# HuiGuanLab/Lite-MKD

Measured on AMD Instinct MI355X. Metric: episodes/sec (5-way 5-shot, 8x224^2 frames), higher is better.
Workload: dtype f32

## Files before the change

### include/lmkd.h

```cpp
#ifndef LMKD_H
#define LMKD_H
#ifdef __cplusplus
extern "C" {
#endif

int lmkd_abi_version(void);
const char* lmkd_last_error(void);
int lmkd_device_check(int device);
int lmkd_set_activation_dtype(int mode);
int lmkd_get_activation_dtype(void);

int lmkd_gemm_f32(char layA, char layB, int M, int N, int K, float alpha, const float* A, long lda, long sA,
                  const float* B, long ldb, long sB, float beta, float* C, long ldc, long sC, const float* bias,
                  int relu, int batch, void* stream);
int lmkd_gemm_set_mode(int mode);
int lmkd_gemm_set_tile(int t);
long lmkd_gemm_ticket_words(void);
int lmkd_gemm_f32_splitk(char layA, char layB, int M, int N, int K, float alpha, const float* A, long lda, long sA,
                         const float* B, long ldb, long sB, float beta, float* C, long ldc, long sC, const float* bias,
                         int relu, int batch, void* workspace, long ws_bytes, unsigned* tickets, void* stream);

long lmkd_conv2d_packed_weight_elems(int Cout, int Cin, int Cs, int KH, int KW, int mode);
int lmkd_conv2d_pack_weights(const float* w_oihw, float* wp, int Cout, int Cin, int Cs, int KH, int KW, int mode ,
                             void* stream);
int lmkd_conv2d_fwd_row_tiles(int N, int H, int W, int Cout, int KH, int KW, int stride, int pad);
int lmkd_conv2d_fwd_row_tiles_cs(int N, int H, int W, int Cs, int Cout, int KH, int KW, int stride, int pad);
int lmkd_set_elementwise_wg_per_cu(int n);
int lmkd_conv_set_compute_dtype(int mode);
typedef struct lmkd_amax_desc {
  const void* x_words;
  const void* dy_words;
  void* out_words;
  const void* ref_words;
  int flags;
} lmkd_amax_desc;
#define LMKD_AMAX_FENCED 1
int lmkd_h2_fence_eval(const void* const* words, void* const* refs, int n, int* flags, void* stream);
long lmkd_conv_h2_fallbacks(void);
int lmkd_amax(const float* x, long n, void* word, void* stream);
long lmkd_amax_words(void);
long lmkd_conv2d_plane_elems(int ncols, int Kp);
long lmkd_conv_h2_launches(void);
int lmkd_conv2d_repack_multi(const float* const* ws, void* const* wfs, const int* dims, int n, void* stream);
int lmkd_conv2d_split_weights(const float* wp, void* wf, int ncols, int Kp, void* stream);
int lmkd_conv_get_compute_dtype(void);
int lmkd_conv_set_wgrad_planes(int on);
int lmkd_conv_set_patch(int on);
int lmkd_conv_set_stem_patch(int on);
int lmkd_conv_set_s2_patch(int on);
int lmkd_conv_set_wgrad_win16(int on);
int lmkd_conv_set_wgrad_stem(int on);
int lmkd_conv_set_wgrad_window(int on);
int lmkd_conv_set_patch16(int on);
int lmkd_conv_set_persistent(int on);
int lmkd_conv_set_xcd_mode(int mode);
int lmkd_conv_set_tile(int id);
int lmkd_conv2d_fwd(const float* x, const float* wp_fwd, float* y, float* stat_partial, int N, int H, int W, int Cs, int Cout,
                    int KH, int KW, int stride, int pad, void* stream);
int lmkd_conv2d_fwd_pre(const float* x_raw, const float* pre_stats, const float* wp_fwd, float* y, float* stat_partial, int N, int H,
                        int W, int Cs, int Cout, int KH, int KW, int stride, int pad, void* stream);
int lmkd_conv2d_fwd_bn(const float* x, const float* wp_fwd, float* y, const float* bn_stats, const float* res , int relu,
                       int N, int H, int W, int Cs, int Cout, int KH, int KW, int stride, int pad, void* stream,
                       const lmkd_amax_desc* amax );
int lmkd_conv2d_bwd_data(const float* dy, const float* wp_dgrad, float* dx, int N, int H, int W, int Cin, int Cout, int KH, int KW,
                         int stride, int pad, int accumulate, void* stream);
int lmkd_conv2d_bwd_data_bn_tiles(int N, int H, int W, int Cin, int Cout, int KH, int KW, int stride, int pad);
int lmkd_conv2d_bwd_data_bn(const float* dy, const float* wp_dgrad, float* dx, const float* bn_x, const float* bn_stats, float* part,
                            int N, int H, int W, int Cin, int Cout, int KH, int KW, int stride, int pad, void* stream);
long lmkd_conv2d_bwd_weight_workspace(int N, int H, int W, int Cs, int Cout, int KH, int KW, int stride, int pad);
int lmkd_conv2d_bwd_weight(const float* x, const float* dy, float* dw_oihw, float* workspace, long ws_bytes, int N, int H, int W,
                           int Cs, int Cin, int Cout, int KH, int KW, int stride, int pad, void* stream);
int lmkd_conv2d_bwd_weight_pre(const float* x_raw, const float* pre_stats, const float* dy, float* dw_oihw, float* workspace,
                               long ws_bytes, int N, int H, int W, int Cs, int Cin, int Cout, int KH, int KW, int stride, int pad,
                               void* stream);

int lmkd_conv2d_plan(int kind, int N, int H, int W, int Cs, int Cin, int Cout, int KH, int KW, int stride, int pad, int* info_host);

int lmkd_conv2d_bwd_weight_acc(const float* x, const float* pre_stats, const float* dy, float* dw_oihw, float* workspace, long ws_bytes,
                               int N, int H, int W, int Cs, int Cin, int Cout, int KH, int KW, int stride, int pad, void* stream);

int lmkd_frames_u8_to_nhwc4(const unsigned char* src, float* dst, const int* crop_y, const int* crop_x, const int* flip, int F, int Hs,
                            int Ws, int H, int W, int frames_per_video, void* stream);
int lmkd_resize_plan(int in_size, int out_size, int* bounds_host, int* coeffs_host);
int lmkd_resize_pass_u8(const unsigned char* src, unsigned char* dst, const int* bounds_dev, const int* coeffs_dev, int ksize, long outer,
                        int n_in, int n_out, long inner, void* stream);
int lmkd_frames_resize_crop_nhwc4(const unsigned char* src, float* dst, const int* bounds_h, const int* coeffs_h, int ksize_h,
                                  const int* bounds_v, const int* coeffs_v, int ksize_v, const int* crop_y, const int* crop_x,
                                  const int* flip, int F, int Hs, int Ws, int Hr, int Wr, int H, int W, int frames_per_video, void* stream);
long lmkd_jpeg_desc_bytes(void);
long lmkd_jpeg_pool_bytes(int n);
const char* lmkd_jpeg_reason(int reason);
int lmkd_jpeg_plan(const unsigned char* data, const long long* offsets, int n, void* descs, void* pool, long pool_cap, long long* info,
                   long long* totals);
int lmkd_jpeg_decode(const unsigned char* data, const void* descs, const void* pool, int n, short* coef, unsigned char* planes,
                     unsigned char* out, int* status, long long max_blocks, long long max_pixels, void* stream);
int lmkd_jpeg_decode_host(const unsigned char* data, const void* descs, const void* pool, int n, short* coef, unsigned char* planes,
                          unsigned char* out, int* status);
int lmkd_nchw3_to_nhwc4(const float* x_nchw, float* y_nhwc4, int N, int H, int W, void* stream, void* amax_words);
long lmkd_ticket_words(void);
// ... 190 lines not shown
```

### lite-mkd_amd/csrc/gemm.hip

```cpp
#include "gemm_core.h"

struct GemmArgs {
  const float* A;
  const float* B;
  float* C;
  const float* bias;
  long lda, ldb, ldc;
  long sA, sB, sC;
  int M, N, K;
  float alpha, beta;
  int relu;
  int splits, k_per;
  float* ws;
  unsigned* tickets;
};

template <class Cfg, bool A_KMAJOR, bool B_KMAJOR>
__global__ __launch_bounds__(LMKD_THREADS) void gemm_kernel(GemmArgs g) {
  using LA = typename std::conditional<A_KMAJOR, LoaderKMajorDense<Cfg::BM>, LoaderMMajorDense<Cfg::BM>>::type;
  using LB = typename std::conditional<B_KMAJOR, LoaderKMajorDense<Cfg::BN>, LoaderMMajorDense<Cfg::BN>>::type;
  __shared__ __attribute__((aligned(16))) float smem[2 * (LA::LDS_FLOATS + LB::LDS_FLOATS)];
  __shared__ int s_last;
  const int m0 = blockIdx.x * Cfg::BM, n0 = blockIdx.y * Cfg::BN;
  const int S = g.splits;
  const long bz = S > 1 ? blockIdx.z / S : blockIdx.z;
  const int ks = S > 1 ? (int)(blockIdx.z - bz * S) : 0;
  const int k0 = ks * g.k_per;
  const int k1 = S > 1 ? (k0 + g.k_per < g.K ? k0 + g.k_per : g.K) : g.K;
  LA la;
  LB lb;
  la.init(g.A + bz * g.sA, g.lda, m0, g.M, k1);
  lb.init(g.B + bz * g.sB, g.ldb, n0, g.N, k1);
  f32x16 acc[Cfg::TM][Cfg::TN];
  const int nk = (k1 - k0 + LMKD_BK - 1) / LMKD_BK;
  auto koff = [k0](int t) { return k0 + t * LMKD_BK; };
  gemm_mainloop<Cfg>(la, lb, nk, koff, koff, smem, acc);

  const int lane = threadIdx.x & 63, wave = threadIdx.x >> 6;
  const int wm = wave / Cfg::WN, wn = wave % Cfg::WN;
  if (S > 1) {
    float* wp = g.ws + (bz * S + ks) * (long)g.M * g.N;
#pragma unroll
    for (int j = 0; j < Cfg::TN; ++j) {
      const int col = n0 + wn * (Cfg::TN * 32) + j * 32 + (lane & 31);
      if (col >= g.N) continue;
#pragma unroll
      for (int i = 0; i < Cfg::TM; ++i)
#pragma unroll
        for (int e = 0; e < 16; ++e) {
          const int row = m0 + wm * (Cfg::TM * 32) + i * 32 + acc_row(e, lane);
          if (row < g.M) __hip_atomic_store(wp + (long)row * g.N + col, acc[i][j][e], __ATOMIC_RELAXED, __HIP_MEMORY_SCOPE_AGENT);
        }
    }
    asm volatile("s_waitcnt vmcnt(0)" ::: "memory");
    __syncthreads();
    unsigned* tk = g.tickets + (bz * gridDim.y + blockIdx.y) * gridDim.x + blockIdx.x;
    if (threadIdx.x == 0) s_last = atomicAdd(tk, 1u) == (unsigned)(S - 1);
    __syncthreads();
    if (!s_last) return;
    asm volatile("" ::: "memory");
    const float* w0 = g.ws + bz * S * (long)g.M * g.N;
#pragma unroll
    for (int j = 0; j < Cfg::TN; ++j) {
      const int col = n0 + wn * (Cfg::TN * 32) + j * 32 + (lane & 31);
#pragma unroll
      for (int i = 0; i < Cfg::TM; ++i)
#pragma unroll
        for (int e = 0; e < 16; ++e) acc[i][j][e] = 0.f;
      if (col >= g.N) continue;
      for (int q = 0; q < S; ++q) {
        const float* wq = w0 + (long)q * g.M * g.N;
#pragma unroll
        for (int i = 0; i < Cfg::TM; ++i)
#pragma unroll
          for (int e = 0; e < 16; ++e) {
            const int row = m0 + wm * (Cfg::TM * 32) + i * 32 + acc_row(e, lane);
            if (row < g.M) acc[i][j][e] += __hip_atomic_load(wq + (long)row * g.N + col, __ATOMIC_RELAXED, __HIP_MEMORY_SCOPE_AGENT);
          }
      }
    }
    if (threadIdx.x == 0) *tk = 0u;
  }
  float* C = g.C + bz * g.sC;
#pragma unroll
  for (int j = 0; j < Cfg::TN; ++j) {
    const int col = n0 + wn * (Cfg::TN * 32) + j * 32 + (lane & 31);
    if (col >= g.N) continue;
    const float bv = g.bias ? g.bias[col] : 0.f;
#pragma unroll
    for (int i = 0; i < Cfg::TM; ++i) {
#pragma unroll
      for (int e = 0; e < 16; ++e) {
        const int row = m0 + wm * (Cfg::TM * 32) + i * 32 + acc_row(e, lane);
        if (row < g.M) {
          float* c = C + (long)row * g.ldc + col;
          float v = g.alpha * acc[i][j][e] + bv;
          if (g.beta != 0.f) v += g.beta * *c;
          if (g.relu) v = fmaxf(v, 0.f);
          *c = v;
        }
      }
    }
  }
}

#include "gemm_x3.h"

static int g_gemm_mode = -1;
static int g_gemm_tile = 0;
extern "C" int lmkd_gemm_set_tile(int t) { g_gemm_tile = t; return LMKD_OK; }
extern "C" int lmkd_gemm_set_mode(int mode) {
  LMKD_REQUIRE(mode >= -1 && mode <= 2, "lmkd_gemm_set_mode: -1 follow the convolutions, 0 fp32 MFMA, 1 fp32 as 3 x bf16, 2 bf16");
  g_gemm_mode = mode;
  return LMKD_OK;
}
extern "C" int lmkd_conv_get_compute_dtype(void);
static inline int gemm_planes(int M, int N, int K) {
  int m = g_gemm_mode;
  if (m < 0) m = lmkd_conv_get_compute_dtype() == 0 ? 0 : 1;
  if (m == 0 || (long)M * N * K < (1L << 18)) return 0;
  return m == 2 ? 1 : 3;
}

template <class Cfg>
static int launch_gemm(const GemmArgs& g, int batch, int ak, int bk, hipStream_t s) {
  dim3 grid(cdiv(g.M, Cfg::BM), cdiv(g.N, Cfg::BN), batch * (g.splits > 1 ? g.splits : 1));
  if (ak && bk) hipLaunchKernelGGL((gemm_kernel<Cfg, true, true>), grid, dim3(LMKD_THREADS), 0, s, g);
  else if (ak && !bk) hipLaunchKernelGGL((gemm_kernel<Cfg, true, false>), grid, dim3(LMKD_THREADS), 0, s, g);
  else if (!ak && bk) hipLaunchKernelGGL((gemm_kernel<Cfg, false, true>), grid, dim3(LMKD_THREADS), 0, s, g);
  else hipLaunchKernelGGL((gemm_kernel<Cfg, false, false>), grid, dim3(LMKD_THREADS), 0, s, g);
  LMKD_CHECK_LAUNCH("lmkd_gemm_f32");
  return LMKD_OK;
}

#define LMKD_GEMM_TICKET_WORDS 4096
extern "C" long lmkd_gemm_ticket_words(void) { return LMKD_GEMM_TICKET_WORDS; }

static void gemm_split_plan(int M, int N, int K, int batch, long ws_bytes, int* splits, int* k_per) {
  *splits = 1;
  *k_per = K;
  const long tiles = (long)cdiv(M, 64) * cdiv(N, 64) * batch;
  if (tiles > 64 || K < 256) return;
  int S = (int)cdiv(768, tiles);
  if (S > 16) S = 16;
  if (S > K / 128) S = K / 128;
  const long per = (long)M * N * batch * sizeof(float);
  if ((long)S * per > ws_bytes) S = (int)(ws_bytes / per);
  if (S < 2) return;
  int kp = cdiv(cdiv(K, S), LMKD_BK) * LMKD_BK;
  *k_per = kp;
  *splits = cdiv(K, kp);
  if (*splits < 2) { *splits = 1; *k_per = K; }
}

static int gemm_impl(char layA, char layB, int M, int N, int K, float alpha, const float* A, long lda, long sA, const float* B, long ldb,
                     long sB, float beta, float* C, long ldc, long sC, const float* bias, int relu, int batch, void* workspace,
                     long ws_bytes, unsigned* tickets, void* stream) {
  LMKD_REQUIRE(layA == 'K' || layA == 'M', "lmkd_gemm_f32: layA must be 'K' or 'M'");
  LMKD_REQUIRE(layB == 'K' || layB == 'N', "lmkd_gemm_f32: layB must be 'K' or 'N'");
  LMKD_REQUIRE(M > 0 && N > 0 && K > 0 && batch > 0, "lmkd_gemm_f32: empty problem M=%d N=%d K=%d batch=%d", M, N, K, batch);
  LMKD_REQUIRE(A && B && C, "lmkd_gemm_f32: null operand");
  LMKD_REQUIRE(aligned16(A) && aligned16(B), "lmkd_gemm_f32: operands must be 16-byte aligned");
  LMKD_REQUIRE(lda % 4 == 0 && ldb % 4 == 0 && sA % 4 == 0 && sB % 4 == 0, "lmkd_gemm_f32: lda/ldb/strides must be multiples of 4");
  if (layA == 'K') LMKD_REQUIRE(K % 4 == 0, "lmkd_gemm_f32: K %% 4 != 0 with K-major A");
  else LMKD_REQUIRE(M % 4 == 0, "lmkd_gemm_f32: M %% 4 != 0 with K-outer A");
  if (layB == 'K') LMKD_REQUIRE(K % 4 == 0, "lmkd_gemm_f32: K %% 4 != 0 with K-major B");
  else LMKD_REQUIRE(N % 4 == 0, "lmkd_gemm_f32: N %% 4 != 0 with K-outer B");
  GemmArgs g;
  g.A = A; g.B = B; g.C = C; g.bias = bias;
  g.lda = lda; g.ldb = ldb; g.ldc = ldc; g.sA = sA; g.sB = sB; g.sC = sC;
  g.M = M; g.N = N; g.K = K; g.alpha = alpha; g.beta = beta; g.relu = relu;
  g.splits = 1; g.k_per = K; g.ws = (float*)workspace; g.tickets = tickets;
  if (workspace && tickets) gemm_split_plan(M, N, K, batch, ws_bytes, &g.splits, &g.k_per);
  hipStream_t s = (hipStream_t)stream;
  const int ak = layA == 'K', bk = layB == 'K';
  const long t128 = (long)cdiv(M, 128) * cdiv(N, 128) * batch;
  if (g.splits == 1) {
    if (const int npl = gemm_planes(M, N, K)) {
      if (g_gemm_tile == 1) return npl == 3 ? launch_gemm_x3<G3Cfg<128, 128, 2, 2>, 3>(g, batch, ak, bk, s) : launch_gemm_x3<G3Cfg<128, 128, 2, 2>, 1>(g, batch, ak, bk, s);
      if (g_gemm_tile == 2) return npl == 3 ? launch_gemm_x3<G3Cfg<64, 128, 1, 4>, 3>(g, batch, ak, bk, s) : launch_gemm_x3<G3Cfg<64, 128, 1, 4>, 1>(g, batch, ak, bk, s);
      return npl == 3 ? launch_gemm_x3<G3Cfg<64, 64, 2, 2>, 3>(g, batch, ak, bk, s) : launch_gemm_x3<G3Cfg<64, 64, 2, 2>, 1>(g, batch, ak, bk, s);
    }
  }
  if (t128 >= 384) return launch_gemm<TileCfg<128, 128, 2, 2>>(g, batch, ak, bk, s);
  return launch_gemm<TileCfg<64, 64, 2, 2>>(g, batch, ak, bk, s);
}

extern "C" int lmkd_gemm_f32(char layA, char layB, int M, int N, int K, float alpha, const float* A, long lda,
                             long sA, const float* B, long ldb, long sB, float beta, float* C, long ldc, long sC,
                             const float* bias, int relu, int batch, void* stream) {
  return gemm_impl(layA, layB, M, N, K, alpha, A, lda, sA, B, ldb, sB, beta, C, ldc, sC, bias, relu, batch, nullptr, 0, nullptr, stream);
}

extern "C" int lmkd_gemm_f32_splitk(char layA, char layB, int M, int N, int K, float alpha, const float* A, long lda, long sA,
                                    const float* B, long ldb, long sB, float beta, float* C, long ldc, long sC, const float* bias,
                                    int relu, int batch, void* workspace, long ws_bytes, unsigned* tickets, void* stream) {
  LMKD_REQUIRE(workspace && tickets && ws_bytes > 0, "lmkd_gemm_f32_splitk: workspace / tickets missing");
  LMKD_REQUIRE(aligned16(workspace), "lmkd_gemm_f32_splitk: workspace must be 16-byte aligned");
  return gemm_impl(layA, layB, M, N, K, alpha, A, lda, sA, B, ldb, sB, beta, C, ldc, sC, bias, relu, batch, workspace, ws_bytes, tickets, stream);
}
```

### lite-mkd_amd/csrc/gemm_core.h

```cpp
#pragma once
#include "common.h"
#include <type_traits>

#define LMKD_BK 32
#define LMKD_THREADS 256

struct Tap {
  int dh, dw, kofs;
};
#define LMKD_MAX_TAPS 9
#define LMKD_MAX_CLASSES 4

template <int BM_, int BN_, int WM_, int WN_>
struct TileCfg {
  static constexpr int BM = BM_, BN = BN_, WM = WM_, WN = WN_;
  static constexpr int TM = BM / WM / 32, TN = BN / WN / 32;
  static constexpr int THREADS = 64 * WM * WN;
  static_assert(WM * WN == 4 || WM * WN == 8, "4 or 8 waves");
  static_assert(TM >= 1 && TN >= 1, "wave tile");
};

#define LMKD_LDK 36

template <int ROWS, int THREADS = LMKD_THREADS>
// ... 114 lines not shown

typedef __bf16 bf16x8 __attribute__((ext_vector_type(8)));

template <bool ROWK, int LD, int N>
__device__ __forceinline__ void read_frags_bf16(const float* __restrict__ S, int row, int h, int m, bf16x8 (&f)[N]) {
#pragma unroll
  for (int i = 0; i < N; ++i) {
    float v[8];
    if (ROWK) {
      const float4 q0 = *reinterpret_cast<const float4*>(S + (row + 32 * i) * LD + 16 * m + 8 * h);
      const float4 q1 = *reinterpret_cast<const float4*>(S + (row + 32 * i) * LD + 16 * m + 8 * h + 4);
      v[0] = q0.x; v[1] = q0.y; v[2] = q0.z; v[3] = q0.w; v[4] = q1.x; v[5] = q1.y; v[6] = q1.z; v[7] = q1.w;
    } else {
#pragma unroll
      for (int j = 0; j < 8; ++j) v[j] = S[(16 * m + 8 * h + j) * LD + row + 32 * i];
    }
#pragma unroll
    for (int j = 0; j < 8; ++j) f[i][j] = (__bf16)v[j];
  }
}

template <class Cfg, class LA, class LB>
__device__ __forceinline__ void mfma_kstep_bf16(const float* __restrict__ As, const float* __restrict__ Bs, int a_row, int b_row,
                                                int h, f32x16 (&acc)[Cfg::TM][Cfg::TN]) {
  constexpr int NM = LMKD_BK / 16;
  bf16x8 a[2][Cfg::TM], b[2][Cfg::TN];
  read_frags_bf16<LA::ROWK, LA::LD, Cfg::TM>(As, a_row, h, 0, a[0]);
  read_frags_bf16<LB::ROWK, LB::LD, Cfg::TN>(Bs, b_row, h, 0, b[0]);
#pragma unroll
  for (int m = 0; m < NM; ++m) {
    const int cur = m & 1, nxt = cur ^ 1;
    if (m + 1 < NM) {
      read_frags_bf16<LA::ROWK, LA::LD, Cfg::TM>(As, a_row, h, m + 1, a[nxt]);
      read_frags_bf16<LB::ROWK, LB::LD, Cfg::TN>(Bs, b_row, h, m + 1, b[nxt]);
    }
#pragma unroll
    for (int i = 0; i < Cfg::TM; ++i)
#pragma unroll
      for (int jj = 0; jj < Cfg::TN; ++jj)
        acc[i][jj] = __builtin_amdgcn_mfma_f32_32x32x16_bf16(a[cur][i], b[cur][jj], acc[i][jj], 0, 0, 0);
  }
}

template <class Cfg, class LA, class LB, class FA, class FB, bool BF16 = false, bool FENCE_STORE = false>
__device__ __forceinline__ void gemm_mainloop(LA& la, LB& lb, int nk, FA koffA, FB koffB, float* smem,
                                              f32x16 (&acc)[Cfg::TM][Cfg::TN]) {
  constexpr int SA = LA::LDS_FLOATS, SB = LB::LDS_FLOATS;
  float* As0 = smem;
  float* Bs0 = smem + 2 * SA;
  const int lane = threadIdx.x & 63, wave = threadIdx.x >> 6;
  const int wm = wave / Cfg::WN, wn = wave % Cfg::WN;
  const int h = lane >> 5;
  const int a_row = wm * (Cfg::TM * 32) + (lane & 31);
  const int b_row = wn * (Cfg::TN * 32) + (lane & 31);
#pragma unroll
  for (int i = 0; i < Cfg::TM; ++i)
#pragma unroll
    for (int j = 0; j < Cfg::TN; ++j)
#pragma unroll
      for (int e = 0; e < 16; ++e) acc[i][j][e] = 0.f;
  if (nk <= 0) return;
  la.load(koffA(0));
  lb.load(koffB(0));
  la.store(As0);
  lb.store(Bs0);
  __syncthreads();
  for (int t = 0; t + 1 < nk; ++t) {
    const int cur = t & 1;
    la.load(koffA(t + 1));
    lb.load(koffB(t + 1));
    if (BF16) mfma_kstep_bf16<Cfg, LA, LB>(As0 + cur * SA, Bs0 + cur * SB, a_row, b_row, h, acc);
    else mfma_kstep<Cfg, LA, LB>(As0 + cur * SA, Bs0 + cur * SB, a_row, b_row, h, acc);
    __builtin_amdgcn_sched_barrier(0);
    (void)FENCE_STORE;
    la.store(As0 + (cur ^ 1) * SA);
    lb.store(Bs0 + (cur ^ 1) * SB);
    __syncthreads();
  }
  const int last = (nk - 1) & 1;
  if (BF16) mfma_kstep_bf16<Cfg, LA, LB>(As0 + last * SA, Bs0 + last * SB, a_row, b_row, h, acc);
  else mfma_kstep<Cfg, LA, LB>(As0 + last * SA, Bs0 + last * SB, a_row, b_row, h, acc);
}

__device__ __forceinline__ int acc_row(int e, int lane) { return (e & 3) + 8 * (e >> 2) + 4 * (lane >> 5); }
```

### lite-mkd_amd/csrc/gemm_x3.h

```cpp
#pragma once

typedef short g3_s16x4 __attribute__((ext_vector_type(4)));
#define G3_LD 40

__device__ __forceinline__ unsigned g3_hi2(unsigned x1, unsigned x0) { return __builtin_amdgcn_perm(x1, x0, 0x07060302u); }

template <int NPL>
__device__ __forceinline__ void g3_split_store(unsigned char* d, int plane_bytes, const float4& v) {
  if (NPL == 1) {
    union { __bf16 h[4]; uint2 u; } c;
    c.h[0] = (__bf16)v.x; c.h[1] = (__bf16)v.y; c.h[2] = (__bf16)v.z; c.h[3] = (__bf16)v.w;
    *reinterpret_cast<uint2*>(d) = c.u;
    return;
  }
  const float x[4] = {v.x, v.y, v.z, v.w};
  unsigned b0[4], b1[4], b2[4];
#pragma unroll
  for (int j = 0; j < 4; ++j) {
    b0[j] = __float_as_uint(x[j]);
    const float r1 = x[j] - __uint_as_float(b0[j] & 0xffff0000u);
    b1[j] = __float_as_uint(r1);
    const float r2 = r1 - __uint_as_float(b1[j] & 0xffff0000u);
    b2[j] = __float_as_uint(r2);
  }
  *reinterpret_cast<uint2*>(d) = make_uint2(g3_hi2(b0[1], b0[0]), g3_hi2(b0[3], b0[2]));
  *reinterpret_cast<uint2*>(d + plane_bytes) = make_uint2(g3_hi2(b1[1], b1[0]), g3_hi2(b1[3], b1[2]));
  *reinterpret_cast<uint2*>(d + 2 * plane_bytes) = make_uint2(g3_hi2(b2[1], b2[0]), g3_hi2(b2[3], b2[2]));
}

template <int ROWS, bool KMAJOR, int NPL>
struct G3Img {
  static constexpr int LDB = KMAJOR ? G3_LD * 2 : ROWS * 2 + 64;
  static constexpr int PLANE = KMAJOR ? ROWS * LDB : LMKD_BK * LDB;
  static constexpr int BYTES = NPL * PLANE;
  static_assert(KMAJOR || (LDB / 64) % 2 == 1, "K-outer row stride must be an odd multiple of 64 bytes");
  template <class L>
  static __device__ __forceinline__ void store(unsigned char* img, const L& l) {
    const int tid = threadIdx.x;
#pragma unroll
    for (int i = 0; i < L::NI; ++i) {
      if constexpr (KMAJOR) g3_split_store<NPL>(img + (((tid >> 3) + L::RPP * i) * G3_LD + l.kc4) * 2, PLANE, l.reg[i]);
      else g3_split_store<NPL>(img + (tid / L::CPR + L::KPP * i) * LDB + l.r4 * 2, PLANE, l.reg[i]);
    }
  }
  static __device__ __forceinline__ int lane_off(int row0, int lane) {
    if (KMAJOR) return ((row0 + (lane & 31)) * G3_LD + 8 * (lane >> 5)) * 2;
    const int idx = lane & 15;
    return (8 * (lane >> 5) + (idx >> 2)) * LDB + (row0 + 16 * ((lane >> 4) & 1) + 4 * (idx & 3)) * 2;
  }
  static __device__ __forceinline__ bf16x8 frag(const unsigned char* img, int off, int i, int g, int p) {
    if (KMAJOR) return *reinterpret_cast<const bf16x8*>(img + off + p * PLANE + i * (32 * LDB) + g * 32);
    const unsigned char* a = img + off + p * PLANE + g * 16 * LDB + i * 64;
    const g3_s16x4 lo = __builtin_amdgcn_ds_read_tr16_b64_v4i16((g3_s16x4 __attribute__((address_space(3)))*)a);
    const g3_s16x4 hi = __builtin_amdgcn_ds_read_tr16_b64_v4i16((g3_s16x4 __attribute__((address_space(3)))*)(a + 4 * LDB));
    union { g3_s16x4 s[2]; bf16x8 b; } u;
    u.s[0] = lo; u.s[1] = hi;
    return u.b;
  }
};

template <int BM_, int BN_, int WM_, int WN_>
struct G3Cfg {
  static constexpr int BM = BM_, BN = BN_, WM = WM_, WN = WN_;
  static constexpr int TM = BM / WM / 32, TN = BN / WN / 32;
  static_assert(WM * WN == 4 && TM >= 1 && TN >= 1, "4 waves");
};

template <class Cfg, bool A_KMAJOR, bool B_KMAJOR, int NPL>
__global__ __launch_bounds__(LMKD_THREADS) void gemm_x3_kernel(GemmArgs g) {
  using LA = typename std::conditional<A_KMAJOR, LoaderKMajorDense<Cfg::BM>, LoaderMMajorDense<Cfg::BM>>::type;
  using LB = typename std::conditional<B_KMAJOR, LoaderKMajorDense<Cfg::BN>, LoaderMMajorDense<Cfg::BN>>::type;
  using IA = G3Img<Cfg::BM, A_KMAJOR, NPL>;
  using IB = G3Img<Cfg::BN, B_KMAJOR, NPL>;
  __shared__ __attribute__((aligned(16))) unsigned char smem[IA::BYTES + IB::BYTES];
  unsigned char* sa = smem;
  unsigned char* sb = smem + IA::BYTES;
  const int m0 = blockIdx.x * Cfg::BM, n0 = blockIdx.y * Cfg::BN;
  const long bz = blockIdx.z;
  LA la;
  LB lb;
  la.init(g.A + bz * g.sA, g.lda, m0, g.M, g.K);
  lb.init(g.B + bz * g.sB, g.ldb, n0, g.N, g.K);
  const int lane = threadIdx.x & 63, wave = threadIdx.x >> 6;
  const int wm = wave / Cfg::WN, wn = wave % Cfg::WN;
  const int offA = IA::lane_off(wm * (Cfg::TM * 32), lane), offB = IB::lane_off(wn * (Cfg::TN * 32), lane);
  f32x16 acc[Cfg::TM][Cfg::TN];
#pragma unroll
  for (int i = 0; i < Cfg::TM; ++i)
#pragma unroll
    for (int j = 0; j < Cfg::TN; ++j)
#pragma unroll
      for (int e = 0; e < 16; ++e) acc[i][j][e] = 0.f;
  unsigned sgn[Cfg::TM];
#pragma unroll
  for (int i = 0; i < Cfg::TM; ++i)
    sgn[i] = (NPL == 3 && (((m0 >> 5) + wm * Cfg::TM + i + (n0 >> 5) + wn * Cfg::TN) & 1)) ? 0x80008000u : 0u;
  const int nk = (g.K + LMKD_BK - 1) / LMKD_BK;
  LA la2 = la;
  LB lb2 = lb;
  auto step = [&](int t, LA& xa, LB& xb) {
      IA::store(sa, xa);
      IB::store(sb, xb);
      __syncthreads();
      if (t + 2 < nk) {
        xa.load((t + 2) * LMKD_BK);
        xb.load((t + 2) * LMKD_BK);
      }
      bf16x8 fa[2][NPL][Cfg::TM], fb[2][NPL][Cfg::TN];
      auto read_group = [&](int gq) {
#pragma unroll
        for (int p = 0; p < NPL; ++p) {
#pragma unroll
          for (int i = 0; i < Cfg::TM; ++i) {
            union { bf16x8 b; unsigned u[4]; } c;
            c.b = IA::frag(sa, offA, i, gq, p);
            if (NPL == 3) { c.u[0] ^= sgn[i]; c.u[1] ^= sgn[i]; c.u[2] ^= sgn[i]; c.u[3] ^= sgn[i]; }
            fa[gq][p][i] = c.b;
          }
#pragma unroll
          for (int j = 0; j < Cfg::TN; ++j) fb[gq][p][j] = IB::frag(sb, offB, j, gq, p);
        }
      };
      read_group(0);
#pragma unroll
      for (int gq = 0; gq < 2; ++gq) {
        if (gq == 0) {
          read_group(1);
          __builtin_amdgcn_sched_barrier(0);
        }
#pragma unroll
        for (int i = 0; i < Cfg::TM; ++i)
#pragma unroll
          for (int j = 0; j < Cfg::TN; ++j) {
            f32x16 c = acc[i][j];
            if constexpr (NPL == 1) {
              c = __builtin_amdgcn_mfma_f32_32x32x16_bf16(fa[gq][0][i], fb[gq][0][j], c, 0, 0, 0);
            } else {
              c = __builtin_amdgcn_mfma_f32_32x32x16_bf16(fa[gq][1][i], fb[gq][1][j], c, 0, 0, 0);
              c = __builtin_amdgcn_mfma_f32_32x32x16_bf16(fa[gq][0][i], fb[gq][2][j], c, 0, 0, 0);
              c = __builtin_amdgcn_mfma_f32_32x32x16_bf16(fa[gq][2][i], fb[gq][0][j], c, 0, 0, 0);
              c = __builtin_amdgcn_mfma_f32_32x32x16_bf16(fa[gq][0][i], fb[gq][1][j], c, 0, 0, 0);
              c = __builtin_amdgcn_mfma_f32_32x32x16_bf16(fa[gq][1][i], fb[gq][0][j], c, 0, 0, 0);
              c = __builtin_amdgcn_mfma_f32_32x32x16_bf16(fa[gq][0][i], fb[gq][0][j], c, 0, 0, 0);
            }
            acc[i][j] = c;
          }
      }
      __syncthreads();
  };
  if (nk > 0) {
    la.load(0);
    lb.load(0);
    if (nk > 1) {
      la2.load(LMKD_BK);
      lb2.load(LMKD_BK);
    }
    int t = 0;
    for (; t + 1 < nk; t += 2) {
      step(t, la, lb);
      step(t + 1, la2, lb2);
    }
    if (t < nk) step(t, la, lb);
  }
  float* C = g.C + bz * g.sC;
#pragma unroll
  for (int j = 0; j < Cfg::TN; ++j) {
    const int col = n0 + wn * (Cfg::TN * 32) + j * 32 + (lane & 31);
    if (col >= g.N) continue;
    const float bv = g.bias ? g.bias[col] : 0.f;
#pragma unroll
    for (int i = 0; i < Cfg::TM; ++i) {
#pragma unroll
      for (int e = 0; e < 16; ++e) {
        const int row = m0 + wm * (Cfg::TM * 32) + i * 32 + acc_row(e, lane);
        if (row < g.M) {
          float* c = C + (long)row * g.ldc + col;
          const float a = sgn[i] ? -acc[i][j][e] : acc[i][j][e];
          float v = g.alpha * a + bv;
          if (g.beta != 0.f) v += g.beta * *c;
          if (g.relu) v = fmaxf(v, 0.f);
          *c = v;
        }
      }
    }
  }
}

template <class Cfg, int NPL>
static int launch_gemm_x3(const GemmArgs& g, int batch, int ak, int bk, hipStream_t s) {
  dim3 grid(cdiv(g.M, Cfg::BM), cdiv(g.N, Cfg::BN), batch);
  if (ak && bk) hipLaunchKernelGGL((gemm_x3_kernel<Cfg, true, true, NPL>), grid, dim3(LMKD_THREADS), 0, s, g);
  else if (ak && !bk) hipLaunchKernelGGL((gemm_x3_kernel<Cfg, true, false, NPL>), grid, dim3(LMKD_THREADS), 0, s, g);
  else if (!ak && bk) hipLaunchKernelGGL((gemm_x3_kernel<Cfg, false, true, NPL>), grid, dim3(LMKD_THREADS), 0, s, g);
  else hipLaunchKernelGGL((gemm_x3_kernel<Cfg, false, false, NPL>), grid, dim3(LMKD_THREADS), 0, s, g);
  LMKD_CHECK_LAUNCH("lmkd_gemm_x3");
  return LMKD_OK;
}
```

Before: 49.71.

## Rework bf16x3 GEMM with XCD-grouped tile order, LDS double buffering, prefetch sets

Adds a 1-D grid with a tile decode that places groups of output tiles on the same XCD (blocks strided by 8), so neighbouring tiles can share L2. The bf16-plane GEMM gets new dedicated loaders with tail handling, a configurable number of register prefetch sets, an optional double-buffered LDS image that overlaps the next tile's store with the current MFMAs, and a 32x64 two-wave tile option. The aim is to hide global and LDS latency and improve cache locality. The cost is larger LDS use that can lower occupancy, more kernel template instantiations, and more complex tail logic.

```diff
diff --git a/include/lmkd.h b/include/lmkd.h
--- a/include/lmkd.h
+++ b/include/lmkd.h
@@ -15,6 +15,10 @@
                   int relu, int batch, void* stream);
 int lmkd_gemm_set_mode(int mode);
 int lmkd_gemm_set_tile(int t);
+int lmkd_gemm_set_order(int order);
+int lmkd_gemm_set_prefetch(int sets);
+int lmkd_gemm_set_images(int images);
+int lmkd_gemm_tile_order(int M, int N, int batch, char layA, char layB, int K, int* out);
 long lmkd_gemm_ticket_words(void);
 int lmkd_gemm_f32_splitk(char layA, char layB, int M, int N, int K, float alpha, const float* A, long lda, long sA,
                          const float* B, long ldb, long sB, float beta, float* C, long ldc, long sC, const float* bias,
diff --git a/lite-mkd_amd/csrc/gemm.hip b/lite-mkd_amd/csrc/gemm.hip
--- a/lite-mkd_amd/csrc/gemm.hip
+++ b/lite-mkd_amd/csrc/gemm.hip
@@ -13,6 +13,7 @@
   int splits, k_per;
   float* ws;
   unsigned* tickets;
+  GemmOrder ord;
 };
 
 template <class Cfg, bool A_KMAJOR, bool B_KMAJOR>
@@ -21,9 +22,11 @@
   using LB = typename std::conditional<B_KMAJOR, LoaderKMajorDense<Cfg::BN>, LoaderMMajorDense<Cfg::BN>>::type;
   __shared__ __attribute__((aligned(16))) float smem[2 * (LA::LDS_FLOATS + LB::LDS_FLOATS)];
   __shared__ int s_last;
-  const int m0 = blockIdx.x * Cfg::BM, n0 = blockIdx.y * Cfg::BN;
   const int S = g.splits;
-  const long bz = S > 1 ? blockIdx.z / S : blockIdx.z;
+  int rt = blockIdx.x, ct = blockIdx.y, bq = S > 1 ? blockIdx.z / S : 0;
+  if (S <= 1 && !gemm_tile_decode(blockIdx.x, g.ord, bq, rt, ct)) return;
+  const int m0 = rt * Cfg::BM, n0 = ct * Cfg::BN;
+  const long bz = bq;
   const int ks = S > 1 ? (int)(blockIdx.z - bz * S) : 0;
   const int k0 = ks * g.k_per;
   const int k1 = S > 1 ? (k0 + g.k_per < g.K ? k0 + g.k_per : g.K) : g.K;
@@ -108,7 +111,29 @@
 
 static int g_gemm_mode = -1;
 static int g_gemm_tile = 0;
-extern "C" int lmkd_gemm_set_tile(int t) { g_gemm_tile = t; return LMKD_OK; }
+static int g_gemm_order = 1;
+static int g_gemm_prefetch = 0;
+extern "C" int lmkd_gemm_set_tile(int t) {
+  LMKD_REQUIRE(t >= 0 && t <= 4, "lmkd_gemm_set_tile: 0 auto, 1 = 128 x 128, 2 = 64 x 128, 3 = 64 x 64, 4 = 32 x 64");
+  g_gemm_tile = t;
+  return LMKD_OK;
+}
+extern "C" int lmkd_gemm_set_order(int order) {
+  LMKD_REQUIRE(order >= 0 && order <= 2, "lmkd_gemm_set_order: 0 plain tile order, 1 XCD-local groups where they are even, 2 groups always");
+  g_gemm_order = order;
+  return LMKD_OK;
+}
+extern "C" int lmkd_gemm_set_prefetch(int sets) {
+  LMKD_REQUIRE(sets == 0 || (sets >= 2 && sets <= 4), "lmkd_gemm_set_prefetch: 0 default, 2 / 3 / 4 loader register sets");
+  g_gemm_prefetch = sets;
+  return LMKD_OK;
+}
+static int g_gemm_images = 0;
+extern "C" int lmkd_gemm_set_images(int images) {
+  LMKD_REQUIRE(images >= 0 && images <= 2, "lmkd_gemm_set_images: 0 default, 1 / 2 LDS tile images");
+  g_gemm_images = images;
+  return LMKD_OK;
+}
 extern "C" int lmkd_gemm_set_mode(int mode) {
   LMKD_REQUIRE(mode >= -1 && mode <= 2, "lmkd_gemm_set_mode: -1 follow the convolutions, 0 fp32 MFMA, 1 fp32 as 3 x bf16, 2 bf16");
   g_gemm_mode = mode;
@@ -124,7 +149,8 @@
 
 template <class Cfg>
 static int launch_gemm(const GemmArgs& g, int batch, int ak, int bk, hipStream_t s) {
-  dim3 grid(cdiv(g.M, Cfg::BM), cdiv(g.N, Cfg::BN), batch * (g.splits > 1 ? g.splits : 1));
+  dim3 grid(gemm_order_grid(g.ord));
+  if (g.splits > 1) grid = dim3(cdiv(g.M, Cfg::BM), cdiv(g.N, Cfg::BN), batch * g.splits);
   if (ak && bk) hipLaunchKernelGGL((gemm_kernel<Cfg, true, true>), grid, dim3(LMKD_THREADS), 0, s, g);
   else if (ak && !bk) hipLaunchKernelGGL((gemm_kernel<Cfg, true, false>), grid, dim3(LMKD_THREADS), 0, s, g);
   else if (!ak && bk) hipLaunchKernelGGL((gemm_kernel<Cfg, false, true>), grid, dim3(LMKD_THREADS), 0, s, g);
@@ -151,6 +177,36 @@
   *k_per = kp;
   *splits = cdiv(K, kp);
   if (*splits < 2) { *splits = 1; *k_per = K; }
+}
+
+struct GemmPlan {
+  int planes;
+  int tile;
+  int images;
+  GemmOrder ord;
+};
+#define LMKD_GEMM_TWO_IMAGES_UPTO 512
+static GemmPlan gemm_plan(int M, int N, int K, int batch, int splits) {
+  GemmPlan p;
+  p.planes = splits == 1 ? gemm_planes(M, N, K) : 0;
+  p.images = 1;
+  int bm = 64, bn = 64;
+  if (p.planes) {
+    p.tile = g_gemm_tile ? g_gemm_tile : 3;
+    p.images = (long)cdiv(M, 64) * cdiv(N, 64) * batch <= LMKD_GEMM_TWO_IMAGES_UPTO ? 2 : 1;
+    if (p.tile == 1) bm = bn = 128;
+    else if (p.tile == 2) bn = 128;
+    else if (p.tile == 4) bm = 32;
+  } else {
+    p.tile = (long)cdiv(M, 128) * cdiv(N, 128) * batch >= 384 ? 1 : 3;
+    if (p.tile == 1) bm = bn = 128;
+  }
+  p.ord.n_rt = cdiv(M, bm);
+  p.ord.n_ct = cdiv(N, bn);
+  p.ord.batch = batch;
+  p.ord.mode = (g_gemm_order == 0 || splits > 1) ? 0 : ((long)N * p.ord.n_rt >= (long)M * p.ord.n_ct ? 1 : 2);
+  if (g_gemm_order == 1 && (batch * (p.ord.mode == 1 ? p.ord.n_ct : p.ord.n_rt)) % 8 != 0) p.ord.mode = 0;
+  return p;
 }
 
 static int gemm_impl(char layA, char layB, int M, int N, int K, float alpha, const float* A, long lda, long sA, const float* B, long ldb,
@@ -174,16 +230,33 @@
   if (workspace && tickets) gemm_split_plan(M, N, K, batch, ws_bytes, &g.splits, &g.k_per);
   hipStream_t s = (hipStream_t)stream;
   const int ak = layA == 'K', bk = layB == 'K';
-  const long t128 = (long)cdiv(M, 128) * cdiv(N, 128) * batch;
-  if (g.splits == 1) {
-    if (const int npl = gemm_planes(M, N, K)) {
-      if (g_gemm_tile == 1) return npl == 3 ? launch_gemm_x3<G3Cfg<128, 128, 2, 2>, 3>(g, batch, ak, bk, s) : launch_gemm_x3<G3Cfg<128, 128, 2, 2>, 1>(g, batch, ak, bk, s);
-      if (g_gemm_tile == 2) return npl == 3 ? launch_gemm_x3<G3Cfg<64, 128, 1, 4>, 3>(g, batch, ak, bk, s) : launch_gemm_x3<G3Cfg<64, 128, 1, 4>, 1>(g, batch, ak, bk, s);
-      return npl == 3 ? launch_gemm_x3<G3Cfg<64, 64, 2, 2>, 3>(g, batch, ak, bk, s) : launch_gemm_x3<G3Cfg<64, 64, 2, 2>, 1>(g, batch, ak, bk, s);
-    }
-  }
-  if (t128 >= 384) return launch_gemm<TileCfg<128, 128, 2, 2>>(g, batch, ak, bk, s);
+  const GemmPlan p = gemm_plan(M, N, K, batch, g.splits);
+  LMKD_REQUIRE((long)p.ord.n_rt * p.ord.n_ct * batch < (1L << 30), "lmkd_gemm_f32: %ld output tiles", (long)p.ord.n_rt * p.ord.n_ct * batch);
+  g.ord = p.ord;
+  if (p.planes) {
+    if (p.tile == 1) return p.planes == 3 ? launch_gemm_x3<G3Cfg<128, 128, 2, 2>, 3, 2>(g, ak, bk, s) : launch_gemm_x3<G3Cfg<128, 128, 2, 2>, 1, 2>(g, ak, bk, s);
+    if (p.tile == 2) return p.planes == 3 ? launch_gemm_x3<G3Cfg<64, 128, 1, 4>, 3, 2>(g, ak, bk, s) : launch_gemm_x3<G3Cfg<64, 128, 1, 4>, 1, 2>(g, ak, bk, s);
+    const int sets = g_gemm_prefetch ? g_gemm_prefetch : LMKD_GEMM_PREFETCH, im = g_gemm_images ? g_gemm_images : p.images;
+    if (p.tile == 4) return p.planes == 3 ? launch_gemm_x3_sets<G3Cfg<32, 64, 1, 2>, 3>(g, ak, bk, sets, im, s) : launch_gemm_x3_sets<G3Cfg<32, 64, 1, 2>, 1>(g, ak, bk, sets, im, s);
+    return p.planes == 3 ? launch_gemm_x3_sets<G3Cfg<64, 64, 2, 2>, 3>(g, ak, bk, sets, im, s) : launch_gemm_x3_sets<G3Cfg<64, 64, 2, 2>, 1>(g, ak, bk, sets, im, s);
+  }
+  if (p.tile == 1) return launch_gemm<TileCfg<128, 128, 2, 2>>(g, batch, ak, bk, s);
   return launch_gemm<TileCfg<64, 64, 2, 2>>(g, batch, ak, bk, s);
+}
+
+extern "C" int lmkd_gemm_tile_order(int M, int N, int batch, char layA, char layB, int K, int* out) {
+  LMKD_REQUIRE(layA == 'K' || layA == 'M', "lmkd_gemm_tile_order: layA must be 'K' or 'M'");
+  LMKD_REQUIRE(layB == 'K' || layB == 'N', "lmkd_gemm_tile_order: layB must be 'K' or 'N'");
+  LMKD_REQUIRE(M > 0 && N > 0 && K > 0 && batch > 0, "lmkd_gemm_tile_order: empty problem M=%d N=%d K=%d batch=%d", M, N, K, batch);
+  const GemmPlan p = gemm_plan(M, N, K, batch, 1);
+  LMKD_REQUIRE((long)p.ord.n_rt * p.ord.n_ct * batch < (1L << 30), "lmkd_gemm_tile_order: %ld output tiles", (long)p.ord.n_rt * p.ord.n_ct * batch);
+  const int blocks = gemm_order_grid(p.ord);
+  for (int b = 0; out && b < blocks; ++b) {
+    int bz, rt, ct;
+    if (!gemm_tile_decode(b, p.ord, bz, rt, ct)) bz = rt = ct = -1;
+    out[3 * b] = bz; out[3 * b + 1] = rt; out[3 * b + 2] = ct;
+  }
+  return blocks;
 }
 
 extern "C" int lmkd_gemm_f32(char layA, char layB, int M, int N, int K, float alpha, const float* A, long lda,
diff --git a/lite-mkd_amd/csrc/gemm_core.h b/lite-mkd_amd/csrc/gemm_core.h
--- a/lite-mkd_amd/csrc/gemm_core.h
+++ b/lite-mkd_amd/csrc/gemm_core.h
@@ -220,4 +220,32 @@
   else mfma_kstep<Cfg, LA, LB>(As0 + last * SA, Bs0 + last * SB, a_row, b_row, h, acc);
 }
 
+struct GemmOrder {
+  int n_rt, n_ct, batch, mode;
+};
+__host__ __device__ __forceinline__ bool gemm_tile_decode(int b, const GemmOrder& o, int& bz, int& rt, int& ct) {
+  if (o.mode == 0) {
+    rt = b % o.n_rt;
+    const int q = b / o.n_rt;
+    ct = q % o.n_ct;
+    bz = q / o.n_ct;
+    return bz < o.batch;
+  }
+  const int gs = o.mode == 1 ? o.n_rt : o.n_ct;
+  const int go = o.mode == 1 ? o.n_ct : o.n_rt;
+  const int j = b >> 3;
+  const int grp = (b & 7) + 8 * (j / gs);
+  const int i = j % gs;
+  bz = grp / go;
+  const int gi = grp - bz * go;
+  rt = o.mode == 1 ? i : gi;
+  ct = o.mode == 1 ? gi : i;
+  return bz < o.batch;
+}
+static inline int gemm_order_grid(const GemmOrder& o) {
+  if (o.mode == 0) return o.n_rt * o.n_ct * o.batch;
+  const int gs = o.mode == 1 ? o.n_rt : o.n_ct, groups = o.batch * (o.mode == 1 ? o.n_ct : o.n_rt);
+  return 8 * gs * ((groups + 7) / 8);
+}
+
 __device__ __forceinline__ int acc_row(int e, int lane) { return (e & 3) + 8 * (e >> 2) + 4 * (lane >> 5); }
diff --git a/lite-mkd_amd/csrc/gemm_x3.h b/lite-mkd_amd/csrc/gemm_x3.h
--- a/lite-mkd_amd/csrc/gemm_x3.h
+++ b/lite-mkd_amd/csrc/gemm_x3.h
@@ -28,19 +28,70 @@
   *reinterpret_cast<uint2*>(d + 2 * plane_bytes) = make_uint2(g3_hi2(b2[1], b2[0]), g3_hi2(b2[3], b2[2]));
 }
 
+template <int ROWS, int THREADS>
+struct G3LoadK {
+  static constexpr int RPP = THREADS / 8, NI = ROWS / RPP;
+  static_assert(ROWS % RPP == 0, "tile rows vs threads");
+  const float* p[NI];
+  float4 reg[NI];
+  int kc4, K;
+  __device__ __forceinline__ void init(const float* base, long ld, int row0, int nrows, int K_) {
+    kc4 = (threadIdx.x & 7) * 4;
+    K = K_;
+#pragma unroll
+    for (int i = 0; i < NI; ++i) {
+      const int r = row0 + (threadIdx.x >> 3) + RPP * i;
+      p[i] = r < nrows ? base + (long)r * ld : base;
+    }
+  }
+  template <bool TAIL>
+  __device__ __forceinline__ void load(int koff) {
+    const int k = (!TAIL || koff + kc4 < K) ? koff + kc4 : 0;
+#pragma unroll
+    for (int i = 0; i < NI; ++i) reg[i] = *reinterpret_cast<const float4*>(p[i] + k);
+  }
+  __device__ __forceinline__ bool valid(int koff, int) const { return koff + kc4 < K; }
+};
+template <int ROWS, int THREADS>
+struct G3LoadM {
+  static constexpr int CPR = ROWS / 4, KPP = THREADS / CPR, NI = LMKD_BK / KPP;
+  static_assert(THREADS % CPR == 0 && LMKD_BK % KPP == 0, "tile rows vs threads");
+  const float* base;
+  long ld;
+  float4 reg[NI];
+  int K, r4, kr;
+  __device__ __forceinline__ void init(const float* base_, long ld_, int row0, int nrows, int K_) {
+    r4 = (threadIdx.x % CPR) * 4;
+    kr = threadIdx.x / CPR;
+    base = (row0 + r4) < nrows ? base_ + row0 + r4 : base_;
+    ld = ld_;
+    K = K_;
+  }
+  template <bool TAIL>
+  __device__ __forceinline__ void load(int koff) {
+#pragma unroll
+    for (int i = 0; i < NI; ++i) {
+      const int k = koff + kr + KPP * i;
+      reg[i] = *reinterpret_cast<const float4*>(base + (long)((!TAIL || k < K) ? k : 0) * ld);
+    }
+  }
+  __device__ __forceinline__ bool valid(int koff, int i) const { return koff + kr + KPP * i < K; }
+};
+
 template <int ROWS, bool KMAJOR, int NPL>
 struct G3Img {
-  static constexpr int LDB = KMAJOR ? G3_LD * 2 : ROWS * 2 + 64;
+  static constexpr int LDB = KMAJOR ? G3_LD * 2 : ROWS * 2 + ((ROWS * 2 / 64) % 2 == 0 ? 64 : 128);
   static constexpr int PLANE = KMAJOR ? ROWS * LDB : LMKD_BK * LDB;
   static constexpr int BYTES = NPL * PLANE;
   static_assert(KMAJOR || (LDB / 64) % 2 == 1, "K-outer row stride must be an odd multiple of 64 bytes");
-  template <class L>
-  static __device__ __forceinline__ void store(unsigned char* img, const L& l) {
+  template <bool TAIL, class L>
+  static __device__ __forceinline__ void store(unsigned char* img, const L& l, int koff) {
     const int tid = threadIdx.x;
 #pragma unroll
     for (int i = 0; i < L::NI; ++i) {
-      if constexpr (KMAJOR) g3_split_store<NPL>(img + (((tid >> 3) + L::RPP * i) * G3_LD + l.kc4) * 2, PLANE, l.reg[i]);
-      else g3_split_store<NPL>(img + (tid / L::CPR + L::KPP * i) * LDB + l.r4 * 2, PLANE, l.reg[i]);
+      const float4 v = (!TAIL || l.valid(koff, i)) ? l.reg[i] : make_float4(0.f, 0.f, 0.f, 0.f);
+      if constexpr (KMAJOR) g3_split_store<NPL>(img + (((tid >> 3) + L::RPP * i) * G3_LD + l.kc4) * 2, PLANE, v);
+      else g3_split_store<NPL>(img + (tid / L::CPR + L::KPP * i) * LDB + l.r4 * 2, PLANE, v);
     }
   }
   static __device__ __forceinline__ int lane_off(int row0, int lane) {
@@ -63,24 +114,30 @@
 struct G3Cfg {
   static constexpr int BM = BM_, BN = BN_, WM = WM_, WN = WN_;
   static constexpr int TM = BM / WM / 32, TN = BN / WN / 32;
-  static_assert(WM * WN == 4 && TM >= 1 && TN >= 1, "4 waves");
+  static constexpr int THREADS = 64 * WM * WN;
+  static_assert((WM * WN == 4 || WM * WN == 2) && TM >= 1 && TN >= 1, "2 or 4 waves");
 };
 
-template <class Cfg, bool A_KMAJOR, bool B_KMAJOR, int NPL>
-__global__ __launch_bounds__(LMKD_THREADS) void gemm_x3_kernel(GemmArgs g) {
-  using LA = typename std::conditional<A_KMAJOR, LoaderKMajorDense<Cfg::BM>, LoaderMMajorDense<Cfg::BM>>::type;
-  using LB = typename std::conditional<B_KMAJOR, LoaderKMajorDense<Cfg::BN>, LoaderMMajorDense<Cfg::BN>>::type;
+#define LMKD_GEMM_PREFETCH 2
+
+template <class Cfg, bool A_KMAJOR, bool B_KMAJOR, int NPL, int NS, bool DB>
+__global__ __launch_bounds__(Cfg::THREADS) void gemm_x3_kernel(GemmArgs g) {
+  using LA = typename std::conditional<A_KMAJOR, G3LoadK<Cfg::BM, Cfg::THREADS>, G3LoadM<Cfg::BM, Cfg::THREADS>>::type;
+  using LB = typename std::conditional<B_KMAJOR, G3LoadK<Cfg::BN, Cfg::THREADS>, G3LoadM<Cfg::BN, Cfg::THREADS>>::type;
   using IA = G3Img<Cfg::BM, A_KMAJOR, NPL>;
   using IB = G3Img<Cfg::BN, B_KMAJOR, NPL>;
-  __shared__ __attribute__((aligned(16))) unsigned char smem[IA::BYTES + IB::BYTES];
+  constexpr int TILE_BYTES = IA::BYTES + IB::BYTES;
+  __shared__ __attribute__((aligned(16))) unsigned char smem[(DB ? 2 : 1) * TILE_BYTES];
   unsigned char* sa = smem;
   unsigned char* sb = smem + IA::BYTES;
-  const int m0 = blockIdx.x * Cfg::BM, n0 = blockIdx.y * Cfg::BN;
-  const long bz = blockIdx.z;
-  LA la;
-  LB lb;
-  la.init(g.A + bz * g.sA, g.lda, m0, g.M, g.K);
-  lb.init(g.B + bz * g.sB, g.ldb, n0, g.N, g.K);
+  int rt, ct, bq;
+  if (!gemm_tile_decode(blockIdx.x, g.ord, bq, rt, ct)) return;
+  const int m0 = rt * Cfg::BM, n0 = ct * Cfg::BN;
+  const long bz = bq;
+  LA la[NS];
+  LB lb[NS];
+  la[0].init(g.A + bz * g.sA, g.lda, m0, g.M, g.K);
+  lb[0].init(g.B + bz * g.sB, g.ldb, n0, g.N, g.K);
   const int lane = threadIdx.x & 63, wave = threadIdx.x >> 6;
   const int wm = wave / Cfg::WN, wn = wave % Cfg::WN;
   const int offA = IA::lane_off(wm * (Cfg::TM * 32), lane), offB = IB::lane_off(wn * (Cfg::TN * 32), lane);
@@ -96,38 +153,33 @@
   for (int i = 0; i < Cfg::TM; ++i)
     sgn[i] = (NPL == 3 && (((m0 >> 5) + wm * Cfg::TM + i + (n0 >> 5) + wn * Cfg::TN) & 1)) ? 0x80008000u : 0u;
   const int nk = (g.K + LMKD_BK - 1) / LMKD_BK;
-  LA la2 = la;
-  LB lb2 = lb;
-  auto step = [&](int t, LA& xa, LB& xb) {
-      IA::store(sa, xa);
-      IB::store(sb, xb);
-      __syncthreads();
-      if (t + 2 < nk) {
-        xa.load((t + 2) * LMKD_BK);
-        xb.load((t + 2) * LMKD_BK);
-      }
+#pragma unroll
+  for (int q = 1; q < NS; ++q) {
+    la[q] = la[0];
+    lb[q] = lb[0];
+  }
+  auto multiply = [&](int buf, auto between) {
+      const unsigned char* ta = sa + buf;
+      const unsigned char* tb = sb + buf;
       bf16x8 fa[2][NPL][Cfg::TM], fb[2][NPL][Cfg::TN];
-      auto read_group = [&](int gq) {
+#pragma unroll
+      for (int gq = 0; gq < 2; ++gq)
 #pragma unroll
         for (int p = 0; p < NPL; ++p) {
 #pragma unroll
           for (int i = 0; i < Cfg::TM; ++i) {
             union { bf16x8 b; unsigned u[4]; } c;
-            c.b = IA::frag(sa, offA, i, gq, p);
+            c.b = IA::frag(ta, offA, i, gq, p);
             if (NPL == 3) { c.u[0] ^= sgn[i]; c.u[1] ^= sgn[i]; c.u[2] ^= sgn[i]; c.u[3] ^= sgn[i]; }
             fa[gq][p][i] = c.b;
           }
 #pragma unroll
-          for (int j = 0; j < Cfg::TN; ++j) fb[gq][p][j] = IB::frag(sb, offB, j, gq, p);
+          for (int j = 0; j < Cfg::TN; ++j) fb[gq][p][j] = IB::frag(tb, offB, j, gq, p);
         }
-      };
-      read_group(0);
-#pragma unroll
-      for (int gq = 0; gq < 2; ++gq) {
-        if (gq == 0) {
-          read_group(1);
-          __builtin_amdgcn_sched_barrier(0);
-        }
+      __builtin_amdgcn_sched_barrier(0);
+      between();
+#pragma unroll
+      for (int gq = 0; gq < 2; ++gq)
 #pragma unroll
         for (int i = 0; i < Cfg::TM; ++i)
 #pragma unroll
@@ -145,22 +197,68 @@
             }
             acc[i][j] = c;
           }
-      }
-      __syncthreads();
   };
-  if (nk > 0) {
-    la.load(0);
-    lb.load(0);
-    if (nk > 1) {
-      la2.load(LMKD_BK);
-      lb2.load(LMKD_BK);
-    }
+  const int full = g.K / LMKD_BK;
+  constexpr std::true_type tail;
+  constexpr std::false_type whole;
+#pragma unroll
+  for (int q = 0; q < NS; ++q) {
+    la[q].template load<true>(q * LMKD_BK);
+    lb[q].template load<true>(q * LMKD_BK);
+  }
+  if constexpr (!DB) {
+    auto step = [&](auto tl, int t, LA& xa, LB& xb) {
+        constexpr bool TAIL = decltype(tl)::value;
+        IA::template store<TAIL>(sa, xa, t * LMKD_BK);
+        IB::template store<TAIL>(sb, xb, t * LMKD_BK);
+        __syncthreads();
+        if (!TAIL || t + NS < nk) {
+          xa.template load<TAIL>((t + NS) * LMKD_BK);
+          xb.template load<TAIL>((t + NS) * LMKD_BK);
+        }
+        multiply(0, [] {});
+        __syncthreads();
+    };
     int t = 0;
-    for (; t + 1 < nk; t += 2) {
-      step(t, la, lb);
-      step(t + 1, la2, lb2);
-    }
-    if (t < nk) step(t, la, lb);
+    for (; t + 2 * NS <= full; t += NS) {
+#pragma unroll
+      for (int q = 0; q < NS; ++q) step(whole, t + q, la[q], lb[q]);
+    }
+    for (; t < nk; t += NS) {
+#pragma unroll
+      for (int q = 0; q < NS; ++q)
+        if (t + q < nk) step(tail, t + q, la[q], lb[q]);
+    }
+  } else if (nk > 0) {
+    IA::template store<true>(sa, la[0], 0);
+    IB::template store<true>(sb, lb[0], 0);
+    la[0].template load<true>(NS * LMKD_BK);
+    lb[0].template load<true>(NS * LMKD_BK);
+    __syncthreads();
+    auto step = [&](auto tl, int t, LA& xa, LB& xb) {
+        constexpr bool TAIL = decltype(tl)::value;
+        const int cur = (t & 1) * TILE_BYTES;
+        multiply(cur, [&] {
+          IA::template store<TAIL>(sa + (TILE_BYTES - cur), xa, (t + 1) * LMKD_BK);
+          IB::template store<TAIL>(sb + (TILE_BYTES - cur), xb, (t + 1) * LMKD_BK);
+        });
+        if (!TAIL || t + 1 + NS < nk) {
+          xa.template load<TAIL>((t + 1 + NS) * LMKD_BK);
+          xb.template load<TAIL>((t + 1 + NS) * LMKD_BK);
+        }
+        __syncthreads();
+    };
+    int t = 0;
+    for (; t + 2 * NS < full; t += NS) {
+#pragma unroll
+      for (int q = 0; q < NS; ++q) step(whole, t + q, la[(q + 1) % NS], lb[(q + 1) % NS]);
+    }
+    for (; t + 1 < nk; t += NS) {
+#pragma unroll
+      for (int q = 0; q < NS; ++q)
+        if (t + q + 1 < nk) step(tail, t + q, la[(q + 1) % NS], lb[(q + 1) % NS]);
+    }
+    multiply(((nk - 1) & 1) * TILE_BYTES, [] {});
   }
   float* C = g.C + bz * g.sC;
 #pragma unroll
@@ -186,13 +284,24 @@
   }
 }
 
-template <class Cfg, int NPL>
-static int launch_gemm_x3(const GemmArgs& g, int batch, int ak, int bk, hipStream_t s) {
-  dim3 grid(cdiv(g.M, Cfg::BM), cdiv(g.N, Cfg::BN), batch);
-  if (ak && bk) hipLaunchKernelGGL((gemm_x3_kernel<Cfg, true, true, NPL>), grid, dim3(LMKD_THREADS), 0, s, g);
-  else if (ak && !bk) hipLaunchKernelGGL((gemm_x3_kernel<Cfg, true, false, NPL>), grid, dim3(LMKD_THREADS), 0, s, g);
-  else if (!ak && bk) hipLaunchKernelGGL((gemm_x3_kernel<Cfg, false, true, NPL>), grid, dim3(LMKD_THREADS), 0, s, g);
-  else hipLaunchKernelGGL((gemm_x3_kernel<Cfg, false, false, NPL>), grid, dim3(LMKD_THREADS), 0, s, g);
+template <class Cfg, int NPL, int NS, bool DB = false>
+static int launch_gemm_x3(const GemmArgs& g, int ak, int bk, hipStream_t s) {
+  const dim3 grid(gemm_order_grid(g.ord)), block(Cfg::THREADS);
+  if (ak && bk) hipLaunchKernelGGL((gemm_x3_kernel<Cfg, true, true, NPL, NS, DB>), grid, block, 0, s, g);
+  else if (ak && !bk) hipLaunchKernelGGL((gemm_x3_kernel<Cfg, true, false, NPL, NS, DB>), grid, block, 0, s, g);
+  else if (!ak && bk) hipLaunchKernelGGL((gemm_x3_kernel<Cfg, false, true, NPL, NS, DB>), grid, block, 0, s, g);
+  else hipLaunchKernelGGL((gemm_x3_kernel<Cfg, false, false, NPL, NS, DB>), grid, block, 0, s, g);
   LMKD_CHECK_LAUNCH("lmkd_gemm_x3");
   return LMKD_OK;
 }
+template <class Cfg, int NPL>
+static int launch_gemm_x3_sets(const GemmArgs& g, int ak, int bk, int sets, int images, hipStream_t s) {
+  if (images == 2) {
+    if (sets == 3) return launch_gemm_x3<Cfg, NPL, 3, true>(g, ak, bk, s);
+    if (sets == 4) return launch_gemm_x3<Cfg, NPL, 4, true>(g, ak, bk, s);
+    return launch_gemm_x3<Cfg, NPL, 2, true>(g, ak, bk, s);
+  }
+  if (sets == 3) return launch_gemm_x3<Cfg, NPL, 3>(g, ak, bk, s);
+  if (sets == 4) return launch_gemm_x3<Cfg, NPL, 4>(g, ak, bk, s);
+  return launch_gemm_x3<Cfg, NPL, 2>(g, ak, bk, s);
+}
```

After: 49.62, median of 2. Within noise of the previous version (-0.2%).
